# CityU-AIM-Group/HTD

Hardware: AMD Instinct MI355X
Metric: images/sec (1333x800) HTD-R50 train step (higher is better)
Workload: dtype f32; 1 GPU; HTD ResNet-50 FPN fp32 train step fwd+bwd+SGD, batch 4/GPU @ 1333x800 (padded 1344x800), random-init weights, 2000 RPN proposals/img, 512 RoIs/img/stage; global_batch=4, parallelism=dp1, stage2_positives=168, proposals=random-init RPN (few positives: the regression branch is nearly idle)

## Files before the change

htd_amd/csrc/conv_x3.hip:

```cpp
#include <algorithm>
#include <mutex>
#include <type_traits>
#include <unordered_map>

#include <stdlib.h>

#include "common.h"

namespace {

using f32x16 = __attribute__((ext_vector_type(16))) float;
using bf16x8 = __attribute__((ext_vector_type(8))) __bf16;
using bf16x2 = __attribute__((ext_vector_type(2))) __bf16;
using f32x2 = __attribute__((ext_vector_type(2))) float;
using f32x4 = __attribute__((ext_vector_type(4))) float;

using f16x8 = __attribute__((ext_vector_type(8))) _Float16;
using f16x2 = __attribute__((ext_vector_type(2))) _Float16;

constexpr int XK = 16;
constexpr int NCH = 6;

struct H2Scale { float s, inv; };
__device__ __forceinline__ H2Scale h2_scale(const float *amax)
// ... 683 lines not shown
    int bbuf = 0, abuf = 0, kx = 0;
    int n1shift = (ky1 - PADY) * p.Wx, n1koff = tap_koff(ky1, cs1);
    int n2shift = (ky2 - PADY) * p.Wx, n2koff = tap_koff(ky2, cs2);
    auto tap = [&](int P, bool TAIL) __attribute__((always_inline)) {
        const bool more = s + 1 < s_end, more2 = s + 2 < s_end;
        if constexpr (H2 && HTD_X3H_FRAG_FIRST) mma_tap(abuf, bbuf, kx, ky * KW, 0);
        const bool issued = issue_b();
        if (!TAIL) {
            if constexpr (KW == 1) {
#pragma unroll
                for (int i = 0; i < NP; ++i) load_pass(ky2, n2koff, i, P * NP + i, more2);
            } else {
                const bool last = kx == KW - 1;
                load_pass(last ? n2shift : n1shift, last ? n2koff : n1koff, last ? 0 : kx + 1, P, last ? more2 : more);
            }
        }
        if constexpr (EARLY) {
            if (TAIL) wait_vm<0>();
            else if (issued) wait_vm<NPT + NI_MIN>();
            else wait_vm<NPT>();
#pragma unroll
            for (int i = 0; i < NPT; ++i) landed(ra[(P ^ 1) * NPT + i]);
            mma_tap(abuf, bbuf, kx, ky * KW, (H2 && HTD_X3H_FRAG_FIRST) ? 1 : 2);
            if constexpr (KW == 1) {
#pragma unroll
                for (int i = 0; i < NP; ++i) store_pass(abuf ^ 1, i, (P ^ 1) * NP + i);
            } else {
                store_pass(abuf ^ 1, kx, P ^ 1);
            }
            constexpr int NM = RB * CB * ((MF16 || H2) ? 3 : 6);
            constexpr int PER = (NPT * 36 + NM - 1) / NM;
            __builtin_amdgcn_sched_group_barrier(0x002, 4, 0);
#pragma unroll
            for (int e = 0; e < NM; ++e) {
                __builtin_amdgcn_sched_group_barrier(0x008, 1, 0);
                __builtin_amdgcn_sched_group_barrier(0x002, PER, 0);
            }
            if (!TAIL) {
                if (DIST >= 2 && issued) wait_vm<NPT + NI_MIN>();
                else wait_vm<NPT>();
            }
        } else {
            mma_tap(abuf, bbuf, kx, ky * KW, (H2 && HTD_X3H_FRAG_FIRST) ? 1 : 2);
            if (TAIL) wait_vm<0>();
            else wait_tap(issued);
#pragma unroll
            for (int i = 0; i < NPT; ++i) landed(ra[(P ^ 1) * NPT + i]);
            if (more) {
                if constexpr (KW == 1) {
#pragma unroll
                    for (int i = 0; i < NP; ++i) store_pass(abuf ^ 1, i, (P ^ 1) * NP + i);
                } else {
                    store_pass(abuf ^ 1, kx, P ^ 1);
                }
            }
        }
        lds_barrier();
        bbuf = bbuf + 1 == NB ? 0 : bbuf + 1;
        if (++kx == KW) {
            kx = 0;
            ++s;
            abuf ^= 1;
            cs = cs1; ky = ky1;
            cs1 = cs2; ky1 = ky2;
            if (++ky2 == p.kh) { ky2 = 0; ++cs2; }
            n1shift = n2shift; n1koff = n2koff;
            n2shift = (ky2 - PADY) * p.Wx;
            n2koff = tap_koff(ky2, cs2);
        }
    };
    const int taps_total = (s_end - s_begin) * KW;
    int t = 0;
#pragma unroll 1
    for (; t + 1 < taps_total; t += 2) {
        tap(0, false);
        tap(1, false);
    }
    if (t < taps_total) tap(0, true);
    wait_vm<0>();
#pragma unroll
    for (int i = 0; i < 2 * NPT; ++i) landed(ra[i]);

    x3_epilogue<WGM, WGN, TM, TN, MF16>(p, acc, lds, m0, n0, part, region_b, split);
}

template <int WGM, int WGN, int TM, int TN, int NS>
constexpr int x3q_occupancy()
{
    constexpr int BM = WGM * TM * 32, BN = WGN * TN * 32;
    constexpr int main_bytes = NS * NCH * (BM + BN) * 16;
    constexpr int epi_bytes = WGM * 32 * (BN + 4) * 4;
    constexpr int by_lds = 163840 / (main_bytes > epi_bytes ? main_bytes : epi_bytes);
    constexpr int by_regs = TM * TN >= 4 ? 3 : 4;
    return by_lds < by_regs ? by_lds : by_regs;
}

template <int WGM, int WGN, int TM, int TN, bool MF16, int NS>
__global__ __launch_bounds__(256, (x3q_occupancy<WGM, WGN, TM, TN, NS>())) void conv_x3q_kernel(X3Params p)
{
    constexpr int BM = WGM * TM * 32, BN = WGN * TN * 32;
    constexpr int A_VEC = NCH * BM, B_VEC = NCH * BN;
    constexpr int MAIN_VEC = NS * (A_VEC + B_VEC);
    constexpr int EPI_VEC = WGM * 32 * (BN + 4) / 4;
    constexpr int LDS_VEC = MAIN_VEC > EPI_VEC ? MAIN_VEC : EPI_VEC;
    __shared__ uint4 lds[LDS_VEC];
    uint4 *const lA = lds, *const lB = lds + NS * A_VEC;
    const unsigned lds_a0 = (unsigned)(size_t)(__attribute__((address_space(3))) void *)lA;
    const unsigned lds_b0 = (unsigned)(size_t)(__attribute__((address_space(3))) void *)lB;

    int bid = blockIdx.x, split = 0, sps = 0;
    bool part = false;
    const bool region_b = bid >= p.tiles_a * p.splits_a;
    if (region_b) {
        const int r = bid - p.tiles_a * p.splits_a;
        bid = p.tiles_a + r / p.splits_b;
        split = r % p.splits_b;
        part = p.splits_b > 1;
        sps = p.sps_b;
    } else if (p.splits_a > 1) {
        split = bid % p.splits_a;
        bid = bid / p.splits_a;
        part = true;
        sps = p.sps_a;
    } else {
        const int q = p.tiles_a / 8, r = p.tiles_a % 8, xcd = bid % 8, idx = bid / 8;
        bid = (xcd < r ? xcd * (q + 1) : r * (q + 1) + (xcd - r) * q) + idx;
    }
    const int tile_m = bid / p.nt, tile_n = bid % p.nt;
    const int64_t m0 = (int64_t)tile_m * BM;
    const int n0 = tile_n * BN;

    const int tid = threadIdx.x, lane = tid & 63, wave = tid >> 6;
    const int wm = wave / WGN, wn = wave % WGN;
    const int frow = lane & 31, fhalf = lane >> 5;
    constexpr int RBLK = MF16 ? 16 : 32;
    constexpr int RB = TM * 32 / RBLK, CB = TN * 32 / RBLK;
    const int lrow = MF16 ? (lane & 15) : frow;
    const int kg = lane >> 4;
    const int a_row = (wm * TM * 32 + lrow) * 16;
    const int a_c0 = (MF16 ? kg * BM * 16 : fhalf * BM * 16) + a_row;
    const int a_c1 = MF16 ? ((kg >> 1) * 4 + (kg & 1)) * BM * 16 + a_row : 0;
    const int b_row = (wn * TN * 32 + lrow) * 16;
    const int b_c0 = (MF16 ? kg * BN * 16 : fhalf * BN * 16) + b_row;
    const int b_c1 = MF16 ? ((1 - (kg >> 1)) * 2 + (kg & 1)) * BN * 16 + b_row : 0;
    const int b_c2 = MF16 ? (((kg >> 1) ? 0 : 4) + (kg & 1)) * BN * 16 + b_row : 0;

    const int total_steps = p.ncs;
    const int s_begin = part ? split * sps : 0;
    const int s_end = part ? min(total_steps, s_begin + sps) : total_steps;

    constexpr int NIA = NCH * BM / 64, NIB = NCH * BN / 64, NI = NIA + NIB, NIW = (NI + 3) / 4;
    const int wave_u = __builtin_amdgcn_readfirstlane(wave);
    const uint4 *src[NIW];
    unsigned dst[NIW], adv[NIW];
#pragma unroll
    for (int k = 0; k < NIW; ++k) {
        const int idx = wave_u + 4 * k;
        if (idx < NIA) {
            const int chunk = idx / (BM / 64), half = idx % (BM / 64);
            src[k] = p.xp + (int64_t)chunk * p.xp_rows + m0 + half * 64 + lane;
            dst[k] = lds_a0 + (unsigned)((chunk * BM + half * 64) * 16);
            adv[k] = (unsigned)(NCH * p.xp_rows);
        } else {
            const int j = (idx < NI ? idx : NIA) - NIA, chunk = j / (BN / 64), half = j % (BN / 64);
            src[k] = p.wp + (int64_t)chunk * p.Cop + n0 + half * 64 + lane;
            dst[k] = lds_b0 + (unsigned)((chunk * BN + half * 64) * 16);
// ... 582 lines not shown
int table_cfg(int64_t M, int Co, int Ci, int taps, int epi)
{
    std::lock_guard<std::mutex> lock(g_xtable_mutex);
    if (g_xtable.empty()) return -1;
    const auto it = g_xtable.find(XKey{M, Co, Ci, taps, epi});
    return it == g_xtable.end() ? -1 : it->second;
}

int choose_cfg(int64_t M, int Co, int Ci, int taps, int epi)
{
    int cfg = forced_cfg();
    if (cfg < 0) cfg = table_cfg(M, Co, Ci, taps, epi);
    if (cfg >= 0) return cfg;
    float best = -1.f;
    static const int cand[4] = {1, 3, 2, 0};
    for (int c : cand) {
        const float sc = cfg_score(c, M, Co);
        if (sc > best * 1.005f) { best = sc; cfg = c; }
    }
    return cfg;
}

static const int g_x3p_mfma = getenv("HTD_X3P_MFMA") ? atoi(getenv("HTD_X3P_MFMA")) : 0;
int x3p_mfma()
{
    if (!g_x3p_tune) return g_x3p_mfma;
    const char *e = getenv("HTD_X3P_MFMA");
    return e ? atoi(e) : 0;
}

int x3p_nb()
{
    if (!g_x3p_tune) return 0;
    const char *e = getenv("HTD_X3P_NB");
    return e ? atoi(e) : 0;
}

template <int TM, int TN, int NB>
void launch_tile_nb(const X3Params &p, int kw, dim3 grid, hipStream_t s)
{
    const int mf = x3p_mfma() ? x3p_mfma() : (kw == 1 ? 16 : 32);
    if (mf == 32) {
        if (kw == 1) hipLaunchKernelGGL((conv_x3p_kernel<2, 2, TM, TN, 1, false, NB>), grid, dim3(256), 0, s, p);
        else hipLaunchKernelGGL((conv_x3p_kernel<2, 2, TM, TN, 3, false, NB>), grid, dim3(256), 0, s, p);
    } else {
        if (kw == 1) hipLaunchKernelGGL((conv_x3p_kernel<2, 2, TM, TN, 1, true, NB>), grid, dim3(256), 0, s, p);
        else hipLaunchKernelGGL((conv_x3p_kernel<2, 2, TM, TN, 3, true, NB>), grid, dim3(256), 0, s, p);
    }
}

template <int TM, int TN>
void launch_tile(const X3Params &p, int kw, dim3 grid, hipStream_t s)
{
#ifdef HTD_X3P_DEEP
    const int nb = x3p_nb();
    if (nb == 3) return launch_tile_nb<TM, TN, 3>(p, kw, grid, s);
    if (nb >= 4) return launch_tile_nb<TM, TN, 4>(p, kw, grid, s);
#endif
    launch_tile_nb<TM, TN, 2>(p, kw, grid, s);
}

static const int g_x3q_mfma = getenv("HTD_X3Q_MFMA") ? atoi(getenv("HTD_X3Q_MFMA")) : 0;
static const int g_x3q_ns = getenv("HTD_X3Q_NS") ? atoi(getenv("HTD_X3Q_NS")) : 0;
int x3q_env(const char *name, int at_load)
{
    if (!g_x3p_tune) return at_load;
    const char *e = getenv(name);
    return e ? atoi(e) : 0;
}

template <int TM, int TN>
void launch_tile_q(const X3Params &p, dim3 grid, hipStream_t s)
{
    const int mf = x3q_env("HTD_X3Q_MFMA", g_x3q_mfma), ns = x3q_env("HTD_X3Q_NS", g_x3q_ns);
    if (mf != 32) {
        if (ns == 3) hipLaunchKernelGGL((conv_x3q_kernel<2, 2, TM, TN, true, 3>), grid, dim3(256), 0, s, p);
        else hipLaunchKernelGGL((conv_x3q_kernel<2, 2, TM, TN, true, 2>), grid, dim3(256), 0, s, p);
    } else {
        if (ns == 3) hipLaunchKernelGGL((conv_x3q_kernel<2, 2, TM, TN, false, 3>), grid, dim3(256), 0, s, p);
        else hipLaunchKernelGGL((conv_x3q_kernel<2, 2, TM, TN, false, 2>), grid, dim3(256), 0, s, p);
    }
}

int launch_x3p(X3Params p, int kw, hipStream_t s, void *workspace)
{
    const int total_steps = p.ncs * p.kh;
    const int epi = (p.residual ? 1 : 0) | (p.mask_src ? 2 : 0) | (p.amax ? 4 : 0);
    const int cfg = choose_cfg(p.M, p.Co, p.Ci, p.kh * kw + (p.ntl > 0 ? 100 : 0), epi);
    const XPlan pl = plan_x3p(cfg, p.M, p.Co, total_steps, kw, workspace != nullptr);
    p.tiles_a = pl.tiles_a; p.splits_a = pl.splits_a; p.sps_a = pl.sps_a; p.splits_b = pl.splits_b; p.sps_b = pl.sps_b;
    p.m_rem0 = pl.m_rem0;
    p.partial = (float *)workspace;
    p.mt = (int)htd::ceil_div(p.M, kXCfg[cfg].bm);
    p.nt = (int)htd::ceil_div(p.Co, kXCfg[cfg].bn);
    HTD_REQUIRE(pl.grid > 0 && pl.grid < (1ll << 31), "conv2d_x3p: bad grid");
    const dim3 grid((unsigned)pl.grid);
    if (p.amax != nullptr && kw == 3) {
        switch (cfg) {
        case 0: hipLaunchKernelGGL((conv_x3p_kernel<2, 2, 1, 1, 3, false, HTD_X3H_NB, true>), grid, dim3(256), 0, s, p); break;
        case 1: hipLaunchKernelGGL((conv_x3p_kernel<2, 2, 2, 2, 3, false, HTD_X3H_NB, true>), grid, dim3(256), 0, s, p); break;
        case 2: hipLaunchKernelGGL((conv_x3p_kernel<2, 2, 2, 1, 3, false, HTD_X3H_NB, true>), grid, dim3(256), 0, s, p); break;
        default: hipLaunchKernelGGL((conv_x3p_kernel<2, 2, 1, 2, 3, false, HTD_X3H_NB, true>), grid, dim3(256), 0, s, p); break;
        }
    } else if (p.amax != nullptr) {
        switch (cfg) {
        case 0: hipLaunchKernelGGL((conv_x3p_kernel<2, 2, 1, 1, 1, false, HTD_X3H_NB, true>), grid, dim3(256), 0, s, p); break;
        case 1: hipLaunchKernelGGL((conv_x3p_kernel<2, 2, 2, 2, 1, false, HTD_X3H_NB, true>), grid, dim3(256), 0, s, p); break;
        case 2: hipLaunchKernelGGL((conv_x3p_kernel<2, 2, 2, 1, 1, false, HTD_X3H_NB, true>), grid, dim3(256), 0, s, p); break;
        default: hipLaunchKernelGGL((conv_x3p_kernel<2, 2, 1, 2, 1, false, HTD_X3H_NB, true>), grid, dim3(256), 0, s, p); break;
        }
    } else if (p.xp != nullptr) {
        switch (cfg) {
        case 0: launch_tile_q<1, 1>(p, grid, s); break;
        case 1: launch_tile_q<2, 2>(p, grid, s); break;
        case 2: launch_tile_q<2, 1>(p, grid, s); break;
        default: launch_tile_q<1, 2>(p, grid, s); break;
        }
    } else {
        switch (cfg) {
        case 0: launch_tile<1, 1>(p, kw, grid, s); break;
        case 1: launch_tile<2, 2>(p, kw, grid, s); break;
        case 2: launch_tile<2, 1>(p, kw, grid, s); break;
        default: launch_tile<1, 2>(p, kw, grid, s); break;
        }
    }
    if (pl.partial_floats > 0) {
        const int64_t rows = (p.splits_a > 1 ? p.m_rem0 : 0) + (p.splits_b > 1 ? p.M - p.m_rem0 : 0);
        if ((p.Co & 3) == 0) {
            const unsigned rb = (unsigned)std::min<int64_t>(htd::ceil_div(rows * (p.Co >> 2), 256), p.amax_out ? 1024 : 4096);
            hipLaunchKernelGGL(conv_x3p_splitk_epilogue_vec_kernel, dim3(rb), dim3(256), 0, s, p);
        } else {
            const unsigned rb = (unsigned)std::min<int64_t>(htd::ceil_div(rows * p.Co, 256), p.amax_out ? 1024 : 4096);
            hipLaunchKernelGGL(conv_x3p_splitk_epilogue_kernel, dim3(rb), dim3(256), 0, s, p);
        }
    }
    return htd::check_launch("conv2d_x3p");
}

bool x3h_strided_ok(int Ci, int Co, int kh, int kw, int stride, int pad)
{
    static const bool on = !(getenv("HTD_X3H_STRIDED") && atoi(getenv("HTD_X3H_STRIDED")) == 0);
    return on && Ci % XK == 0 && Co >= 33 && kh == 3 && kw == 3 && stride == 2 && pad == 1;
}

bool x3p_shape_ok(int Ci, int Co, int kh, int kw, int stride, int pad, int dil)
{
    if (Ci % XK != 0 || Co < 33 || dil != 1 || kh != kw) return false;
    if (kh == 1) return pad == 0 && stride >= 1;
    return kh == 3 && stride == 1 && pad == 1;
}

}

extern "C" int htd_conv2d_x3p_supported(int Ci, int Co, int kh, int kw, int stride, int pad, int dil)
{
    return (!x3p_off() && htd::conv_math() == 1 && x3p_shape_ok(Ci, Co, kh, kw, stride, pad, dil)) ? 1 : 0;
}

int g_conv_h2 = getenv("HTD_CONV_H2") ? atoi(getenv("HTD_CONV_H2")) : 1;
extern "C" int htd_conv2d_set_h2(int on)
{
    const int prev = g_conv_h2;
    if (on == 0 || on == 1) g_conv_h2 = on;
    return prev;
}
extern "C" int htd_conv2d_x3h_supported(int Ci, int Co, int kh, int kw, int stride, int pad, int dil)
{
    return (g_conv_h2 == 1 && htd_conv2d_x3p_supported(Ci, Co, kh, kw, stride, pad, dil)) ? 1 : 0;
}
extern "C" int htd_conv2d_x3h_strided_supported(int Ci, int Co, int kh, int kw, int stride, int pad, int dil)
{
    return (g_conv_h2 == 1 && !x3p_off() && htd::conv_math() == 1 && dil == 1 && x3h_strided_ok(Ci, Co, kh, kw, stride, pad)) ? 1 : 0;
}

extern "C" int htd_conv2d_x3p_tile_table_set(int64_t M, int Co, int Ci, int taps, int epi, int cfg)
{
    HTD_REQUIRE(M > 0 && Co > 0 && Ci > 0 && taps > 0 && epi >= 0 && epi < 8 && cfg < 4,
                "x3p_tile_table_set: bad entry M=%lld Co=%d Ci=%d taps=%d epi=%d cfg=%d", (long long)M, Co, Ci, taps, epi, cfg);
    std::lock_guard<std::mutex> lock(g_xtable_mutex);
    if (cfg < 0) g_xtable.erase(XKey{M, Co, Ci, taps, epi});
    else g_xtable[XKey{M, Co, Ci, taps, epi}] = cfg;
    return HTD_OK;
}

extern "C" int htd_conv2d_x3p_tile_table_clear()
{
    std::lock_guard<std::mutex> lock(g_xtable_mutex);
    g_xtable.clear();
    return HTD_OK;
}

extern "C" int htd_conv2d_x3p_tile_query(int64_t M, int Co, int Ci, int taps, int epi)
{
    return choose_cfg(M, Co, Ci, taps, epi);
}

extern "C" int htd_conv2d_x3p_plan_query(int cfg, int64_t M, int Co, int Ci, int kh, int kw, int64_t *out)
{
    HTD_REQUIRE(cfg >= 0 && cfg < 4 && M > 0 && Co > 0 && Ci >= XK && Ci % XK == 0 && kh > 0 && kw > 0 && out,
                "x3p_plan_query: bad arguments");
    const XPlan pl = plan_x3p(cfg, M, Co, (Ci / XK) * kh, kw, true);
    out[0] = pl.tiles_a; out[1] = pl.splits_a; out[2] = pl.sps_a; out[3] = pl.splits_b; out[4] = pl.sps_b;
    out[5] = pl.m_rem0; out[6] = pl.grid; out[7] = pl.partial_floats;
    return HTD_OK;
}

extern "C" int64_t htd_conv2d_x3_planes_bytes(int Co, int kh, int kw, int Ci, int transposed)
{
    const int N = transposed ? Ci : Co, K = transposed ? Co : Ci;
    if (N <= 0 || K <= 0 || K % XK != 0 || kh <= 0 || kw <= 0) return 0;
    return (int64_t)kh * kw * (K / XK) * NCH * planes_np(N) * 16 + (int64_t)(2 + h2_chunks(kh * kw, K)) * planes_np(N) * 4;
}

extern "C" int htd_conv2d_x3_planes(const float *w, void *planes, int Co, int kh, int kw, int Ci, int transposed, void *stream)
{
    HTD_REQUIRE(w && planes && Co > 0 && Ci > 0 && kh > 0 && kw > 0, "x3_planes: bad arguments");
    const int N = transposed ? Ci : Co, K = transposed ? Co : Ci;
    HTD_REQUIRE(K % XK == 0, "x3_planes: reduction length %d must be a multiple of 16", K);
    HTD_REQUIRE(transposed || Ci % 4 == 0, "x3_planes: Ci %% 4");
    const int Np = planes_np(N);
    const int64_t total = (int64_t)kh * kw * (K / XK) * Np;
    const unsigned blocks = (unsigned)std::min<int64_t>(htd::ceil_div(total, 256), 16384);
    hipLaunchKernelGGL(x3_planes_kernel, dim3(blocks), dim3(256), 0, (hipStream_t)stream, w, (uint4 *)planes, Co, kh * kw, Ci, Np,
                       transposed);
    return htd::check_launch("x3_planes");
}

extern "C" int htd_conv2d_x3h_planes(const float *w, void *planes, int Co, int kh, int kw, int Ci, int transposed, void *stream)
{
    HTD_REQUIRE(w && planes && Co > 0 && Ci > 0 && kh > 0 && kw > 0, "x3h_planes: bad arguments");
    const int N = transposed ? Ci : Co, K = transposed ? Co : Ci;
    HTD_REQUIRE(K % XK == 0, "x3h_planes: reduction length %d must be a multiple of 16", K);
    HTD_REQUIRE(transposed || Ci % 4 == 0, "x3h_planes: Ci %% 4");
    const int Np = planes_np(N);
    float *scales = reinterpret_cast<float *>((uint4 *)planes + planes_vec(kh * kw, K, Np));
    hipLaunchKernelGGL(x3h_rowscale_kernel, dim3((unsigned)(Np / 64 * h2_chunks(kh * kw, K))), dim3(256), 0, (hipStream_t)stream, w,
                       scales, Co, kh * kw, Ci, Np, transposed);
    const int64_t total = (int64_t)kh * kw * (K / XK) * Np;
    const unsigned blocks = (unsigned)std::min<int64_t>(htd::ceil_div(total, 256), 16384);
    hipLaunchKernelGGL(x3h_planes_kernel, dim3(blocks), dim3(256), 0, (hipStream_t)stream, w, (uint4 *)planes, scales, Co, kh * kw,
                       Ci, Np, transposed);
    return htd::check_launch("x3h_planes");
}

extern "C" int htd_conv2d_x3h_planes_many(const void *desc, int n, int64_t total_blocks, int64_t total_rows, void *stream)
{
// ... 274 lines not shown
```

include/htd_amd.h:

```cpp
#ifndef HTD_AMD_H
#define HTD_AMD_H

#include <stdint.h>

#ifdef __cplusplus
extern "C" {
#endif

#define HTD_OK 0
#define HTD_ERR_ARG 1
#define HTD_ERR_LAUNCH 2

const char *htd_last_error(void);
#define HTD_ABI_VERSION 7
int htd_abi_version(void);

int htd_roi_align_fwd(const float *feat, const float *rois, const int64_t *roi_level, int level,
                      float *out, int64_t n, int B, int C, int H, int W, int ph, int pw, float spatial_scale,
                      int sampling_ratio, int aligned, void *stream);
int htd_roi_align_bwd(const float *grad_out, const float *rois, const int64_t *roi_level, int level,
                      float *grad_feat, int64_t n, int B, int C, int H, int W, int ph, int pw,
                      float spatial_scale, int sampling_ratio, int aligned, void *stream);
int htd_roi_align_levels_fwd(const float *const *feats, const int *H, const int *W, const float *scales, int L,
                             const float *rois, const int64_t *roi_level, float *out, int64_t n, int B, int C, int ph, int pw,
// ... 47 lines not shown
                      unsigned char *neg_mask, int64_t *counts, int64_t *order, int slots, void *workspace, void *stream);

int htd_fuse_global_fwd(const float *roi_feats, const float *rois, const float *global_feat,
                        const float *extra, float alpha, float *out, int64_t n, int P, int C,
                        int B, void *stream);
int htd_plain_and_fused_fwd(const float *roi_feats, const float *rois, const float *global_feat, float *both,
                            int64_t n, int P, int C, int B, void *stream);
int htd_fuse_global_fwd_amax(const float *roi_feats, const float *rois, const float *global_feat, const float *extra,
                             float alpha, float *out, int64_t n, int P, int C, int B, float *amax_out, void *stream);
int htd_plain_and_fused_fwd_amax(const float *roi_feats, const float *rois, const float *global_feat, float *both,
                                 int64_t n, int P, int C, int B, float *amax_out, void *stream);
int htd_fuse_global_bwd_global(const float *grad, const float *rois, float *grad_global,
                               int64_t n, int P, int C, int B, void *stream);

int htd_ba_fuse_fwd(const float *const *lvl, int L, const float *border, const float *att,
                    float *out, int64_t n, int ph, int pw, int C, int edge, void *stream);
int htd_ba_fuse_bwd(const float *const *lvl, int L, const float *att, const float *grad_out,
                    float *const *grad_lvl, float *grad_border, float *grad_att, int64_t n, int ph,
                    int pw, int C, int edge, void *stream);

int64_t htd_conv2d_workspace_bytes(int64_t M, int Co, int Ci, int kh, int kw);
int htd_conv2d_set_math(int mode);
int htd_conv2d_tile_table_set(int64_t M, int Co, int Ci, int taps, int epi, int cfg);
int htd_conv2d_tile_table_clear(void);
int htd_conv2d_tile_query(int64_t M, int Co, int Ci, int taps, int epi);
int htd_conv2d_fwd(const float *x, const float *w, const float *bias, const float *residual, int res_h,
                   int res_w, float *y, int B, int H, int W, int Ci, int Co, int kh, int kw, int stride,
                   int pad, int dil, int relu, void *workspace, void *stream);
int htd_bgemm_nt(const float *a, const float *b, float *c, int G, int M, int N, int K, void *stream);
int htd_bgemm_nt_counts(const float *a, const float *b, float *c, int G, int M, int N, int K, const int64_t *counts, int limit,
                        void *stream);
int htd_conv2d_flip_weights(const float *w, float *wT, int Co, int kh, int kw, int Ci, void *stream);
int htd_conv2d_flip_weights_padded(const float *w, float *wT, int Co, int Co_padded, int kh, int kw, int Ci, void *stream);
int htd_pad_channels(const float *x, float *y, int64_t rows, int C, int C_padded, void *stream);
int htd_conv2d_bwd_data(const float *gy, const float *wT, const float *mask_src, const float *accum, float *gx,
                        int B, int H, int W, int Ci, int Co, int kh, int kw, int stride, int pad, int dil,
                        void *workspace, void *stream);
int htd_conv2d_fwd_amax(const float *x, const float *w, const float *bias, const float *residual, int res_h, int res_w,
                        float *y, float *amax_out, int B, int H, int W, int Ci, int Co, int kh, int kw, int stride, int pad,
                        int dil, int relu, void *workspace, void *stream);
int htd_conv2d_bwd_data_amax(const float *gy, const float *wT, const float *mask_src, const float *accum, float *gx,
                             float *amax_out, int B, int H, int W, int Ci, int Co, int kh, int kw, int stride, int pad,
                             int dil, void *workspace, void *stream);
int64_t htd_conv2d_wgrad_workspace_bytes(int B, int H, int W, int Ci, int Co, int kh, int kw,
                                         int stride, int pad, int dil);
int htd_conv2d_bwd_weight(const float *x, const float *gy, float *gw, float *gbias, int B, int H, int W,
                          int Ci, int Co, int kh, int kw, int stride, int pad, int dil, void *workspace,
                          void *stream);
int htd_conv2d_bwd_weight_acc(const float *x, const float *gy, float *gw, float *gbias, int B, int H, int W, int Ci,
                              int Co, int kh, int kw, int stride, int pad, int dil, void *workspace, void *stream);
int htd_bias_grad_relu_mask(const float *g, const float *y, float *gm, float *gbias, int64_t rows,
                            int C, void *workspace, void *stream);
int htd_bias_grad_relu_mask_amax(const float *g, const float *y, float *gm, float *gbias, int64_t rows, int C,
                                 void *workspace, float *amax_out, void *stream);
int64_t htd_conv2d_stem7_workspace_bytes(void);
int htd_conv2d_stem7_fwd(const float *x, const float *w, const float *bias, float *y, int B, int H, int W, int relu,
                         void *workspace, void *stream);
int htd_conv2d_x3p_supported(int Ci, int Co, int kh, int kw, int stride, int pad, int dil);
int htd_conv2d_x3p_tile_table_set(int64_t M, int Co, int Ci, int taps, int epi, int cfg);
int htd_conv2d_x3p_tile_table_clear(void);
int htd_conv2d_x3p_tile_query(int64_t M, int Co, int Ci, int taps, int epi);
int htd_conv2d_x3p_plan_query(int cfg, int64_t M, int Co, int Ci, int kh, int kw, int64_t *out);
int64_t htd_conv2d_x3_planes_bytes(int Co, int kh, int kw, int Ci, int transposed);
int htd_conv2d_x3_planes(const float *w, void *planes, int Co, int kh, int kw, int Ci, int transposed, void *stream);
int htd_conv2d_x3_planes_many(const void *desc, int n, int64_t total_blocks, void *stream);
int64_t htd_conv2d_x3p_workspace_bytes(int64_t M, int Co, int Ci, int kh, int kw);
int htd_conv2d_fwd_x3p(const float *x, const void *wplanes, const float *bias, const float *residual, int res_h,
                       int res_w, float *y, int B, int H, int W, int Ci, int Co, int kh, int kw, int stride, int pad,
                       int relu, void *workspace, void *stream);
int htd_conv2d_bwd_data_x3p(const float *gy, const void *wplanesT, const float *mask_src, const float *accum,
                            float *gx, int B, int H, int W, int Ci, int Co, int kh, int kw, int pad, void *workspace,
                            void *stream);
int64_t htd_act_planes_rows(int64_t M);
int64_t htd_act_planes_bytes(int64_t M, int C);
int htd_act_planes(const float *x, void *planes, int64_t M, int C, void *stream);
int htd_conv2d_fwd_x3q(const float *x, const void *xplanes, const void *wplanes, const float *bias, const float *residual,
                       int res_h, int res_w, float *y, void *yplanes, float *amax_out, int B, int H, int W, int Ci, int Co, int kh, int kw,
                       int stride, int pad, int relu, void *workspace, void *stream);
int htd_conv2d_bwd_data_x3q(const float *gy, const void *gyplanes, const void *wplanesT, const float *mask_src,
                            const float *accum, float *gx, void *gxplanes, float *amax_out, int B, int H, int W, int Ci, int Co, int kh, int kw,
                            int pad, void *workspace, void *stream);

int htd_conv2d_set_h2(int on);
int htd_conv2d_bwd_weight_h2_supported(int B, int H, int W, int Ci, int Co, int kh, int kw, int stride, int pad, int dil);
int htd_conv2d_bwd_weight_h2(const float *x, const float *gy, const float *amax_x, const float *amax_g, float *gw,
                             float *gbias, int B, int H, int W, int Ci, int Co, int kh, int kw, int stride, int pad,
                             int dil, int accumulate, void *workspace, void *stream);
int htd_conv2d_x3h_supported(int Ci, int Co, int kh, int kw, int stride, int pad, int dil);
int htd_conv2d_x3h_strided_supported(int Ci, int Co, int kh, int kw, int stride, int pad, int dil);
int htd_conv2d_bwd_data_x3h_strided_supported(int Ci, int Co, int kh, int kw, int stride, int pad, int dil);
int64_t htd_conv2d_bwd_data_x3h_strided_workspace_bytes(int B, int H, int W, int Ci, int Co, int kh, int kw, int stride, int pad);
int htd_conv2d_bwd_data_x3h_strided(const float *gy, const float *amax, const void *wplanesT, const float *mask_src, float *gx,
                                    float *amax_out, int B, int H, int W, int Ci, int Co, int kh, int kw, int stride, int pad,
                                    void *workspace, void *stream);
int htd_absmax(const float *x, int64_t n, float *amax, void *stream);
int htd_conv2d_x3h_planes(const float *w, void *planes, int Co, int kh, int kw, int Ci, int transposed, void *stream);
int htd_conv2d_x3h_planes_many(const void *desc, int n, int64_t total_blocks, int64_t total_rows, void *stream);
int htd_conv2d_fwd_x3h(const float *x, const float *amax, const void *wplanes, const float *bias, const float *residual,
                       int res_h, int res_w, float *y, void *yplanes, float *amax_out, int B, int H, int W, int Ci,
                       int Co, int kh, int kw, int stride, int pad, int relu, void *workspace, void *stream);
int htd_conv2d_bwd_data_x3h(const float *gy, const float *amax, const void *wplanesT, const float *mask_src,
                            const float *accum, float *gx, void *gxplanes, float *amax_out, int B, int H, int W,
                            int Ci, int Co, int kh, int kw, int pad, void *workspace, void *stream);

int64_t htd_deform_columns_bytes(int B, int H, int W, int C, int kh, int kw, int stride, int pad, int dil);
int htd_deform_im2col(const float *x, const float *offset, const float *mask, float *columns, int B,
                      int H, int W, int C, int kh, int kw, int stride, int pad, int dil,
                      int deform_groups, void *stream);
int htd_deform_col2im(const float *x, const float *offset, const float *mask, const float *gcolumns,
                      float *gx, float *goffset, float *gmask, int B, int H, int W, int C, int kh,
                      int kw, int stride, int pad, int dil, int deform_groups, void *stream);
int htd_deform_im2col_bf16(const void *x, const float *offset, const float *mask, void *columns, int B, int H, int W,
                           int C, int kh, int kw, int stride, int pad, int dil, int deform_groups, void *stream);
int htd_deform_col2im_bf16(const void *x, const float *offset, const float *mask, const void *gcolumns, float *gx,
                           float *goffset, float *gmask, int B, int H, int W, int C, int kh, int kw, int stride, int pad,
                           int dil, int deform_groups, void *stream);

int htd_global_avg_pool_fwd(const float *x, float *out, int64_t B, int P, int C, void *stream);
int htd_global_avg_pool_bwd(const float *g, float *gx, int64_t B, int P, int C, void *stream);
int htd_global_avg_pool_bwd_acc(const float *g, float *gx, int64_t B, int P, int C, void *stream);

int htd_group_norm_relu_fwd(const float *x, const float *gamma, const float *beta, float *y,
                            float *mean, float *rstd, int64_t n, int P, int C, int G, float eps,
                            int relu, void *stream);
int htd_group_norm_relu_bwd(const float *x, const float *y, const float *gamma, const float *mean,
                            const float *rstd, const float *gy, float *gx, float *ggamma,
                            float *gbeta, int64_t n, int P, int C, int G, int relu, void *stream);
int htd_group_norm_relu_bwd_ws(const float *x, const float *y, const float *gamma, const float *mean, const float *rstd,
                               const float *gy, float *gx, float *ggamma, float *gbeta, int64_t n, int P, int C, int G,
                               int relu, void *workspace, void *stream);
int htd_group_norm_relu_fwd_amax(const float *x, const float *gamma, const float *beta, float *y, float *mean, float *rstd,
                                 int64_t n, int P, int C, int G, float eps, int relu, float *amax_out, void *stream);
int htd_group_norm_bwd_amax_supported(int P, int C, int G);
int htd_group_norm_relu_bwd_amax(const float *x, const float *y, const float *gamma, const float *mean, const float *rstd,
                                 const float *gy, float *gx, float *ggamma, float *gbeta, int64_t n, int P, int C, int G,
                                 int relu, void *workspace, float *amax_out, void *stream);
int htd_fuse_global_bwd_global_ws(const float *grad, const float *rois, float *grad_global, int64_t n, int P, int C, int B,
                                  void *workspace, void *stream);

int htd_bn_fold_fwd(const float *w, const float *gamma, const float *beta, const float *mean,
                    const float *var, float eps, float *w_folded, float *b_folded, int Co, int K,
                    void *stream);
int htd_bn_fold_bwd(const float *w, const float *gamma, const float *mean, const float *var, float eps,
                    const float *gw_folded, const float *gb_folded, float *gw, float *ggamma,
                    float *gbeta, int Co, int K, void *stream);
int htd_bn_fold_many_fwd(const void *desc, int n_layers, int total_tiles, float eps, void *stream);
int htd_bn_fold_many_bwd(const void *desc, int n_layers, int total_rows, float eps, void *stream);

int64_t htd_max_iou_assign_workspace_bytes(int B, int A, int K);
int htd_max_iou_assign(const float *boxes, int box_shared, const uint8_t *box_valid, const float *gts,
                       const uint8_t *gt_valid, int B, int A, int K, float pos_iou_thr, float neg_iou_thr,
                       float min_pos_iou, int match_low_quality, int64_t *assigned, float *max_overlaps,
                       void *workspace, void *stream);

int htd_roi_targets(const float *boxes, const float *gt_boxes, const int64_t *gt_labels, const uint8_t *is_pos,
                    const uint8_t *valid, int64_t n, int num_classes, const float *means4, const float *stds4,
                    int64_t *labels, float *label_weights, float *bbox_targets, float *bbox_weights, void *stream);
int htd_delta2bbox_clip(const float *rois, const float *deltas, const float *lim_wh, const uint8_t *keep, int64_t n,
                        int64_t rows_per_img, const float *means4, const float *stds4, float wh_ratio_clip,
                        float *out, void *stream);
int htd_map_roi_levels(const float *rois, int64_t *lvls, int64_t n, int num_levels, float finest_scale, void *stream);
int htd_rpn_heads_gather(const float *const *y, const int64_t *pix, int L, int B, int C, int na, float *cls, float *reg,
                         void *stream);
int htd_rpn_heads_scatter(const float *gcls, const float *greg, float *const *gy, const int64_t *pix, int L, int B, int C,
                          int na, void *stream);
int htd_static_samples_finish(const float *gts, const uint8_t *gvalid, const int64_t *glabels, const float *props,
// ... 133 lines not shown
```

Measured before the change: 124.6 images/sec.

## Add wide-K 1x1 split-fp16 conv kernel staging 32/64 channels per barrier

```diff
diff --git a/htd_amd/csrc/conv_x3.hip b/htd_amd/csrc/conv_x3.hip
--- a/htd_amd/csrc/conv_x3.hip
+++ b/htd_amd/csrc/conv_x3.hip
@@ -789,6 +789,220 @@
     for (int i = 0; i < 2 * NPT; ++i) landed(ra[i]);
 
     x3_epilogue<WGM, WGN, TM, TN, MF16>(p, acc, lds, m0, n0, part, region_b, split);
+}
+
+template <int WGM, int WGN, int TM, int TN, int KS>
+struct GeoW {
+    static constexpr int BM = WGM * TM * 32, BN = WGN * TN * 32;
+    static constexpr int PITCH = Geo<BM, 1>::PITCH;
+    static constexpr int A_SL = 4 * PITCH + (KS == 4 ? 1 : 2);
+    static constexpr int A_VEC = KS * A_SL, B_SL = 4 * BN, B_VEC = KS * B_SL;
+    static constexpr int MAIN_VEC = 2 * (A_VEC + B_VEC);
+    static constexpr int EPI_VEC = WGM * 32 * (BN + 4) / 4;
+    static constexpr int LDS_VEC = MAIN_VEC > EPI_VEC ? MAIN_VEC : EPI_VEC;
+    static constexpr int by_lds = 163840 / (LDS_VEC * 16);
+    static constexpr int by_regs = TM * TN >= 4 ? 2 : (TM * TN == 2 ? 3 : 4);
+    static constexpr int OCC = by_lds < by_regs ? by_lds : by_regs;
+};
+
+template <int WGM, int WGN, int TM, int TN, int KS>
+__global__ __launch_bounds__(256, (GeoW<WGM, WGN, TM, TN, KS>::OCC)) void conv_x3w_kernel(X3Params p)
+{
+    static_assert(KS == 2 || KS == 4, "32 or 64 channels per step");
+    using G = GeoW<WGM, WGN, TM, TN, KS>;
+    constexpr int BM = G::BM, BN = G::BN, PITCH = G::PITCH, A_SL = G::A_SL, A_VEC = G::A_VEC, B_SL = G::B_SL, B_VEC = G::B_VEC;
+    __shared__ uint4 lds[G::LDS_VEC];
+    uint4 *const lA = lds, *const lB = lds + 2 * A_VEC;
+    const unsigned lds_a0 = (unsigned)(size_t)(__attribute__((address_space(3))) void *)lA;
+    const unsigned lds_b0 = (unsigned)(size_t)(__attribute__((address_space(3))) void *)lB;
+
+    int bid = blockIdx.x, split = 0, sps = 0;
+    bool part = false;
+    const bool region_b = bid >= p.tiles_a * p.splits_a;
+    if (region_b) {
+        const int r = bid - p.tiles_a * p.splits_a;
+        bid = p.tiles_a + r / p.splits_b;
+        split = r % p.splits_b;
+        part = p.splits_b > 1;
+        sps = p.sps_b;
+    } else if (p.splits_a > 1) {
+        split = bid % p.splits_a;
+        bid = bid / p.splits_a;
+        part = true;
+        sps = p.sps_a;
+    } else {
+        const int q = p.tiles_a / 8, r = p.tiles_a % 8, xcd = bid % 8, idx = bid / 8;
+        bid = (xcd < r ? xcd * (q + 1) : r * (q + 1) + (xcd - r) * q) + idx;
+    }
+    const int tile_m = bid / p.nt, tile_n = bid % p.nt;
+    const int64_t m0 = (int64_t)tile_m * BM;
+    const int n0 = tile_n * BN;
+    const int s_begin = part ? split * sps : 0;
+    const int s_end = part ? min(p.ncs, s_begin + sps) : p.ncs;
+    const int nsteps = (s_end - s_begin + KS - 1) / KS;
+
+    const int tid = threadIdx.x, lane = tid & 63, wave = tid >> 6;
+    const int wm = wave / WGN, wn = wave % WGN;
+    const int frow = lane & 31, fhalf = lane >> 5;
+
+    constexpr int TPR = 4 * KS, RPP = 256 / TPR, NP = BM / RPP;
+    const int vcol = tid & 3, ks = (tid % TPR) >> 2, vrow = tid / TPR;
+    unsigned a_off[NP];
+    unsigned a_in = 0u;
+#pragma unroll
+    for (int i = 0; i < NP; ++i) {
+        const int64_t m = m0 + vrow + RPP * i;
+        const bool in = m < p.M;
+        const unsigned mm = in ? (unsigned)m : 0u;
+        const unsigned wo = mm % (unsigned)p.Wo, t = mm / (unsigned)p.Wo;
+        const unsigned ho = t % (unsigned)p.Ho, b = t / (unsigned)p.Ho;
+        a_off[i] = ((b * (unsigned)p.Hx + ho * (unsigned)p.stride) * (unsigned)p.Wx + wo * (unsigned)p.stride) * (unsigned)p.Ci +
+                   (unsigned)(ks * XK + vcol * 4);
+        a_in |= in ? (1u << i) : 0u;
+    }
+    f32x4 ra[2 * NP];
+#pragma unroll
+    for (int i = 0; i < 2 * NP; ++i) ra[i] = f32x4{0.f, 0.f, 0.f, 0.f};
+    unsigned ra_ok = 0u;
+    const float h2s = h2_scale(p.amax).s;
+    auto load_pass = [&](int cb, int i, int slot) __attribute__((always_inline)) {
+        const bool ok = ((a_in >> i) & 1u) && cb + ks < s_end;
+        const unsigned off = a_off[i] + (unsigned)(cb * XK);
+        ra_ok = ok ? (ra_ok | (1u << slot)) : (ra_ok & ~(1u << slot));
+        asm volatile("global_load_dwordx4 %0, %1, off" : "+v"(ra[slot]) : "v"(p.x + (off & (0u - (unsigned)ok))) : "memory");
+    };
+    auto store_pass = [&](int buf, int i, int slot) __attribute__((always_inline)) {
+        const bool ok = (ra_ok >> slot) & 1u;
+        const float4 v = make_float4(ok ? ra[slot][0] : 0.f, ok ? ra[slot][1] : 0.f, ok ? ra[slot][2] : 0.f, ok ? ra[slot][3] : 0.f);
+        const unsigned d = lds_a0 + (unsigned)((buf * A_VEC + ks * A_SL + (vcol >> 1) * PITCH + vrow + RPP * i) * 16 + (vcol & 1) * 8);
+        unsigned h0, l0, h1, l1;
+        split2hx2(v.x * h2s, v.y * h2s, h0, l0);
+        split2hx2(v.z * h2s, v.w * h2s, h1, l1);
+        lds_store8<0>(d, h0, h1);
+        lds_store8<2 * PITCH * 16>(d, l0, l1);
+    };
+
+    constexpr int NI = 4 * BN / 64, NIW = NI / 4;
+    static_assert(NI % 4 == 0, "every wave issues the same number of LDS-DMA per tile");
+    const uint4 *bsrc[NIW];
+#pragma unroll
+    for (int k = 0; k < NIW; ++k) {
+        const int idx = wave + 4 * k;
+        bsrc[k] = p.wp + (int64_t)(idx / (BN / 64)) * p.Cop + (idx % (BN / 64)) * 64 + n0 + lane;
+    }
+    const int wave_u = __builtin_amdgcn_readfirstlane(wave);
+    const unsigned tile_stride = (unsigned)(NCH * p.Cop);
+    auto load_b = [&](int cb, int buf) __attribute__((always_inline)) {
+#pragma unroll
+        for (int q = 0; q < KS; ++q) {
+            const unsigned tile_off = (unsigned)min(cb + q, s_end - 1) * tile_stride;
+#pragma unroll
+            for (int k = 0; k < NIW; ++k)
+                lds_dma16(bsrc[k] + tile_off, lds_b0 + (unsigned)((buf * B_VEC + q * B_SL + (wave_u + 4 * k) * 64) * 16));
+        }
+    };
+    constexpr int NBW = KS * NIW;
+    auto lds_barrier = [&]() {
+        asm volatile("s_waitcnt lgkmcnt(0)" ::: "memory");
+        __builtin_amdgcn_s_barrier();
+        asm volatile("" ::: "memory");
+    };
+
+    f32x16 acc[TM][TN];
+#pragma unroll
+    for (int i = 0; i < TM; ++i)
+#pragma unroll
+        for (int j = 0; j < TN; ++j)
+#pragma unroll
+            for (int r = 0; r < 16; ++r) acc[i][j][r] = 0.f;
+
+    const int a_frag = ((wm * TM * 32 + frow) + fhalf * PITCH) * 16;
+    const int b_frag = ((wn * TN * 32 + frow) + fhalf * BN) * 16;
+    auto frags = [&](int buf, int q, f16x8 (&fa)[TM][2], f16x8 (&fb)[TN][2]) __attribute__((always_inline)) {
+        const char *la = reinterpret_cast<const char *>(lA + buf * A_VEC + q * A_SL) + a_frag;
+        const char *lb = reinterpret_cast<const char *>(lB + buf * B_VEC + q * B_SL) + b_frag;
+#pragma unroll
+        for (int i = 0; i < TM; ++i)
+#pragma unroll
+            for (int h = 0; h < 2; ++h) fa[i][h] = *reinterpret_cast<const f16x8 *>(la + (i * 32 + h * 2 * PITCH) * 16);
+#pragma unroll
+        for (int j = 0; j < TN; ++j)
+#pragma unroll
+            for (int h = 0; h < 2; ++h) fb[j][h] = *reinterpret_cast<const f16x8 *>(lb + (j * 32 + h * 2 * BN) * 16);
+    };
+    auto mma = [&](const f16x8 (&fa)[TM][2], const f16x8 (&fb)[TN][2]) __attribute__((always_inline)) {
+#pragma unroll
+        for (int i = 0; i < TM; ++i)
+#pragma unroll
+            for (int j = 0; j < TN; ++j) {
+                acc[i][j] = __builtin_amdgcn_mfma_f32_32x32x16_f16(fa[i][1], fb[j][0], acc[i][j], 0, 0, 0);
+                acc[i][j] = __builtin_amdgcn_mfma_f32_32x32x16_f16(fa[i][0], fb[j][1], acc[i][j], 0, 0, 0);
+                acc[i][j] = __builtin_amdgcn_mfma_f32_32x32x16_f16(fa[i][0], fb[j][0], acc[i][j], 0, 0, 0);
+            }
+    };
+
+    int cb = s_begin;
+    load_b(cb, 0);
+#pragma unroll
+    for (int i = 0; i < NP; ++i) load_pass(cb, i, i);
+    wait_vm<0>();
+#pragma unroll
+    for (int i = 0; i < NP; ++i) landed(ra[i]);
+#pragma unroll
+    for (int i = 0; i < NP; ++i) store_pass(0, i, i);
+#pragma unroll
+    for (int i = 0; i < NP; ++i) load_pass(cb + KS, i, NP + i);
+    lds_barrier();
+
+    auto step = [&](int P) __attribute__((always_inline)) {
+        f16x8 fa[2][TM][2], fb[2][TN][2];
+        frags(P, 0, fa[0], fb[0]);
+        load_b(cb + KS, P ^ 1);
+#pragma unroll
+        for (int i = 0; i < NP; ++i) load_pass(cb + 2 * KS, i, P * NP + i);
+#pragma unroll
+        for (int q = 0; q < KS; ++q) {
+            if (q + 1 < KS) frags(P, q + 1, fa[(q + 1) & 1], fb[(q + 1) & 1]);
+            if (q == KS - 1) {
+                wait_vm<NBW + NP>();
+#pragma unroll
+                for (int i = 0; i < NP; ++i) landed(ra[(P ^ 1) * NP + i]);
+            }
+            mma(fa[q & 1], fb[q & 1]);
+        }
+#pragma unroll
+        for (int i = 0; i < NP; ++i) store_pass(P ^ 1, i, (P ^ 1) * NP + i);
+        wait_vm<NP>();
+        lds_barrier();
+        cb += KS;
+    };
+    int j = 0;
+#pragma unroll 1
+    for (; j + 2 < nsteps; j += 2) {
+        step(0);
+        step(1);
+    }
+    if (j + 1 < nsteps) {
+        step(0);
+        ++j;
+    }
+    {
+        const int buf = j & 1, nl = s_end - cb;
+        f16x8 fa[TM][2], fb[TN][2];
+#pragma unroll
+        for (int q = 0; q < KS; ++q) {
+            if (q < nl) {
+                frags(buf, q, fa, fb);
+                mma(fa, fb);
+            }
+        }
+    }
+    wait_vm<0>();
+#pragma unroll
+    for (int i = 0; i < 2 * NP; ++i) landed(ra[i]);
+    __syncthreads();
+
+    x3_epilogue<WGM, WGN, TM, TN, false>(p, acc, lds, m0, n0, part, region_b, split);
 }
 
 template <int WGM, int WGN, int TM, int TN, int NS>
@@ -1537,6 +1751,36 @@
     }
 }
 
+int g_x3h_wide = getenv("HTD_X3H_WIDE") ? (atoi(getenv("HTD_X3H_WIDE")) != 0 ? 1 : 0) : 1;
+int x3h_wide() { return g_x3h_wide; }
+
+constexpr int kXwKS[4] = {4, 2, 2, 2};
+bool x3w_takes(const X3Params &p, int cfg) { return !(cfg == 1 && p.ncs <= 8 && p.M >= 65536); }
+void launch_x3w(const X3Params &p, int cfg, dim3 grid, hipStream_t s)
+{
+    int ks = kXwKS[cfg];
+    if (g_x3p_tune) {
+        const char *e = getenv("HTD_X3W_KS");
+        const int v = e ? atoi(e) : 0;
+        if (v == 2 || v == 4) ks = v;
+    }
+    if (ks == 4) {
+        switch (cfg) {
+        case 0: hipLaunchKernelGGL((conv_x3w_kernel<2, 2, 1, 1, 4>), grid, dim3(256), 0, s, p); break;
+        case 1: hipLaunchKernelGGL((conv_x3w_kernel<2, 2, 2, 2, 4>), grid, dim3(256), 0, s, p); break;
+        case 2: hipLaunchKernelGGL((conv_x3w_kernel<2, 2, 2, 1, 4>), grid, dim3(256), 0, s, p); break;
+        default: hipLaunchKernelGGL((conv_x3w_kernel<2, 2, 1, 2, 4>), grid, dim3(256), 0, s, p); break;
+        }
+    } else {
+        switch (cfg) {
+        case 0: hipLaunchKernelGGL((conv_x3w_kernel<2, 2, 1, 1, 2>), grid, dim3(256), 0, s, p); break;
+        case 1: hipLaunchKernelGGL((conv_x3w_kernel<2, 2, 2, 2, 2>), grid, dim3(256), 0, s, p); break;
+        case 2: hipLaunchKernelGGL((conv_x3w_kernel<2, 2, 2, 1, 2>), grid, dim3(256), 0, s, p); break;
+        default: hipLaunchKernelGGL((conv_x3w_kernel<2, 2, 1, 2, 2>), grid, dim3(256), 0, s, p); break;
+        }
+    }
+}
+
 int launch_x3p(X3Params p, int kw, hipStream_t s, void *workspace)
 {
     const int total_steps = p.ncs * p.kh;
@@ -1557,6 +1801,8 @@
         case 2: hipLaunchKernelGGL((conv_x3p_kernel<2, 2, 2, 1, 3, false, HTD_X3H_NB, true>), grid, dim3(256), 0, s, p); break;
         default: hipLaunchKernelGGL((conv_x3p_kernel<2, 2, 1, 2, 3, false, HTD_X3H_NB, true>), grid, dim3(256), 0, s, p); break;
         }
+    } else if (p.amax != nullptr && p.ntl == 0 && x3h_wide() == 1 && x3w_takes(p, cfg)) {
+        launch_x3w(p, cfg, grid, s);
     } else if (p.amax != nullptr) {
         switch (cfg) {
         case 0: hipLaunchKernelGGL((conv_x3p_kernel<2, 2, 1, 1, 1, false, HTD_X3H_NB, true>), grid, dim3(256), 0, s, p); break;
@@ -1617,6 +1863,12 @@
 {
     const int prev = g_conv_h2;
     if (on == 0 || on == 1) g_conv_h2 = on;
+    return prev;
+}
+extern "C" int htd_conv2d_x3h_set_wide(int on)
+{
+    const int prev = g_x3h_wide;
+    if (on == 0 || on == 1) g_x3h_wide = on;
     return prev;
 }
 extern "C" int htd_conv2d_x3h_supported(int Ci, int Co, int kh, int kw, int stride, int pad, int dil)
diff --git a/include/htd_amd.h b/include/htd_amd.h
--- a/include/htd_amd.h
+++ b/include/htd_amd.h
@@ -153,6 +153,7 @@
                             int pad, void *workspace, void *stream);
 
 int htd_conv2d_set_h2(int on);
+int htd_conv2d_x3h_set_wide(int on);
 int htd_conv2d_bwd_weight_h2_supported(int B, int H, int W, int Ci, int Co, int kh, int kw, int stride, int pad, int dil);
 int htd_conv2d_bwd_weight_h2(const float *x, const float *gy, const float *amax_x, const float *amax_g, float *gw,
                              float *gbias, int B, int H, int W, int Ci, int Co, int kh, int kw, int stride, int pad,
```

Result: slower. 119.1 images/sec (-4.4%).
